# sahaRatul/sela

Hardware: AMD Instinct MI355X
Metric: Msamples/s encode+decode, 16-bit stereo 44.1kHz, 1/2/4/8 GPU; bit-exact vs CPU (higher is better)
Workload: dtype f64+int64

## Files before the change

### sela_amd/csrc/sela_encode.hip

```cpp
#include <algorithm>
#include <atomic>
#include <random>
#include <vector>

#include "sela_device.h"

namespace sela {

constexpr int kPadC = 64;
constexpr int kHalfEntries = kBlock / 4;
constexpr int kParityLen = kPadC + kHalfEntries + 64;
constexpr int kLastT0 = (kHalfEntries + 64) / 32 - 1;
constexpr int kFirstT1 = (kHalfEntries - kPadC) / 32;
constexpr int kRingHalf = 64;
constexpr int kRingLen = 2 * kRingHalf + 64;
constexpr int kRingsPerXcd = 512;
constexpr int kXcds = 8;
constexpr int kPadS = 128;
constexpr int kSBufWords = (kPadS + kBlock) / 32 * 33;
constexpr int kSmallBase = 8992;
constexpr int kBigBytes = kSmallBase + 3008;
static_assert(kResWordsCap * 4 <= kSmallBase, "packed residue words must fit the dead sample buffer");
static_assert(kSBufWords * 4 <= kSmallBase && kSmallBase % 16 == 0, "sample buffer must end below the analysis arrays");
static_assert(kBigBytes >= 2 * kParityLen * 8, "the FP64 parity arrays must fit");
// ... 909 lines not shown
#pragma unroll
    for (int t = 0; t <= kLastT0; t++)
        mine[half + 32 * t] = scale_sample(s[t]);
    wave_sync();

    __builtin_amdgcn_s_setprio(3);
    double sum = 0.0;
#pragma unroll 1
    for (int h = 0; h < 2; h++) {
        if (h == 1) {
            wave_sync();
#pragma unroll
            for (int t = kFirstT1; t < kPerLane; t++)
                mine1[half + 32 * t] = scale_sample(s[t]);
            wave_sync();
        }
        uint32_t addr = (uint32_t)(uintptr_t)(__attribute__((address_space(3))) double*)E;
        MeanFetch f0, f1;
        SELA_MEAN_ISSUE(f0, addr, 0, sum);
#pragma unroll 1
        for (int m0 = 0; m0 < kHalfEntries; m0 += 16) {
            mean_wait(f0, sum);
            SELA_MEAN_ISSUE(f1, addr, 64, sum);
            mean_steps(f0, sum);
            mean_wait(f1, sum);
            SELA_MEAN_ISSUE(f0, addr, 128, sum);
            mean_steps(f1, sum);
            addr += 128;
        }
        mean_wait(f0, sum);
    }
    mean = sum / (double)kBlock;
    __builtin_amdgcn_s_setprio(0);
    }

    SELA_STAMP(2);
    wave_sync();
    for (int m = lane; m < kPadC; m += 64) {
        E[m - kPadC] = 0.0;
        O[m - kPadC] = 0.0;
    }
#pragma unroll
    for (int t = 0; t <= kLastT0; t++)
        mine[half + 32 * t] = scale_sample(s[t]) - mean;
    wave_sync();

    SELA_STAMP(3);
    double acc_e = 0.0, acc_o = 0.0;
    {
        uint32_t xcc;
        asm volatile("s_getreg_b32 %0, hwreg(HW_REG_XCC_ID)" : "=s"(xcc));
        xcc &= kXcds - 1;
        uint32_t* const pool = ring_owner + xcc * kRingsPerXcd;
        uint32_t slot = 0;
        if (lane == 0) {
            slot = (e >> 3) & (kRingsPerXcd - 1);
            while (atomicExch(pool + slot, ticket) == ticket)
                slot = (slot + 1) & (kRingsPerXcd - 1);
        }
        slot = (uint32_t)__builtin_amdgcn_readfirstlane((int)slot);
        double* const ring = reinterpret_cast<double*>(
            read_first_lane((uint64_t)(rings + ((size_t)xcc * kRingsPerXcd + slot) * kRingLen)));
        __attribute__((address_space(1))) double* const ring_g = (__attribute__((address_space(1))) double*)ring;
        auto store_chunk = [&](int k, const double* resident) {
#pragma unroll
            for (int t = 0; t < kRingHalf / 64; t++) {
                const double c = resident[half + 32 * (t + (kRingHalf / 64) * k)];
                ring_g[(k & 1) * kRingHalf + lane + 64 * t] = c;
                if (t == 0 && !(k & 1) && lane < 16)
                    ring_g[2 * kRingHalf + lane] = c;
            }
        };
        store_chunk(0, mine);
        store_chunk(1, mine);
        asm volatile("s_waitcnt vmcnt(0)\n\ts_dcache_inv" ::: "memory");

        double A = E[-lane];
        double B = 0.0;
        uint32_t addr_e = (uint32_t)(uintptr_t)(__attribute__((address_space(3))) double*)(E - lane);
        uint32_t addr_o = (uint32_t)(uintptr_t)(__attribute__((address_space(3))) double*)(O - lane);
        const double* c_ptr = ring;
        AcFetch f0, f1;
        asm volatile("" : "+v"(A));
        SELA_AC_ISSUE_S(f0, c_ptr, 0, 64, acc_e, acc_o);
        SELA_AC_ISSUE_V(f0, addr_e, addr_o, 0, 1, 2, 3, 4, 5, 6, 7, 8, acc_e, acc_o);
        constexpr int kSwitch = kBlock / 2 / kRingHalf;
        const bool falling = !kFused && n_workers == 0 && fa.priorities != 0;
#pragma unroll 1
        for (int k = 0; k < kBlock / kRingHalf; k++) {
            if (falling && k == 0)
                __builtin_amdgcn_s_setprio(2);
            if (falling && k == kSwitch)
                __builtin_amdgcn_s_setprio(1);
            if (k == kSwitch) {
                wave_sync();
#pragma unroll
                for (int t = kFirstT1; t < kPerLane; t++)
                    mine1[half + 32 * t] = scale_sample(s[t]) - mean;
                wave_sync();
                addr_e -= kHalfEntries * 8;
                addr_o -= kHalfEntries * 8;
            }
            if (k >= 1 && k + 1 < kBlock / kRingHalf)
                store_chunk(k + 1, k >= kSwitch ? mine1 : mine);
#pragma unroll 1
            for (int it = 0; it < kRingHalf / 32; it++) {
                if (it == kRingHalf / 32 - 1)
                    asm volatile("s_waitcnt vmcnt(0)\n\ts_dcache_inv" ::: "memory");
                ac_wait(f0, acc_e, acc_o);
                SELA_AC_ISSUE_S(f1, c_ptr, 128, 192, acc_e, acc_o);
                ac_steps_head(f0, A, B, acc_e, acc_o);
                SELA_AC_ISSUE_V(f1, addr_e, addr_o, 8, 9, 10, 11, 12, 13, 14, 15, 16, acc_e, acc_o);
                ac_steps_tail(f0, A, B, acc_e, acc_o);
                ac_wait(f1, acc_e, acc_o);
                SELA_AC_ISSUE_S(f0, c_ptr, 256, 320, acc_e, acc_o);
                ac_steps_head(f1, A, B, acc_e, acc_o);
                SELA_AC_ISSUE_V(f0, addr_e, addr_o, 16, 17, 18, 19, 20, 21, 22, 23, 24, acc_e, acc_o);
                ac_steps_tail(f1, A, B, acc_e, acc_o);
                c_ptr += 32;
                addr_e += 128;
                addr_o += 128;
            }
            if (k & 1)
                c_ptr = ring;
        }
        ac_wait(f0, acc_e, acc_o);
        if (lane == 0)
            atomicExch(pool + slot, 0u);
    }
    wave_sync();

    SELA_STAMP(4);
    {
        const double ac0 = read_first_lane(acc_e);
        if (lane <= 50) {
            sm->ac[2 * lane] = lane == 0 ? 1.0 : acc_e / ac0;
            sm->ac[2 * lane + 1] = acc_o / ac0;
        }
    }
    wave_sync();

    double k_lo = 0.0, k_hi = 0.0;
    if (!kFused && n_workers == 0 && fa.priorities != 0)
        __builtin_amdgcn_s_setprio(1);
    else
        __builtin_amdgcn_s_setprio(2);
    {
        double g0a = sm->ac[lane + 1], g1a = g0a;
        double g0b = lane < 36 ? sm->ac[lane + 65] : 0.0, g1b = g0b;
        double err = 1.0;
        double g = read_first_lane(g1a);
        double ki = -g / err;
        err += g * ki;
        sm->k[0] = ki;
        constexpr int kTwoRegs = kMaxOrder - 64 + 1;
#pragma unroll 1
        for (int i = 1; i < kTwoRegs; i++) {
            const double sa = wave_shl1(read_first_lane(g1b), g1a);
            const double sb = wave_shl1_zero(g1b);
            g1a = sa + ki * g0a;
            g0a = sa * ki + g0a;
            g1b = sb + ki * g0b;
            g0b = sb * ki + g0b;
            g = read_first_lane(g1a);
            ki = -g / err;
            err += g * ki;
            sm->k[i] = ki;
        }
#pragma unroll 1
        for (int i = kTwoRegs; i < kMaxOrder; i++) {
            const double sa = wave_shl1_zero(g1a);
            g1a = sa + ki * g0a;
            g0a = sa * ki + g0a;
            g = read_first_lane(g1a);
            ki = -g / err;
            err += g * ki;
            sm->k[i] = ki;
        }
        wave_sync();
        k_lo = sm->k[lane];
        k_hi = lane < kMaxOrder - 64 ? sm->k[lane + 64] : 0.0;
        wave_sync();
    }
    if (kMode == 3) {
        uint64_t h_ac = hash_term(sm->ac[lane], lane) ^ (lane + 64 <= kMaxOrder ? hash_term(sm->ac[lane + 64], lane + 64) : 0ull);
        uint64_t h_k = hash_term(k_lo, lane) ^ (lane < kMaxOrder - 64 ? hash_term(k_hi, lane + 64) : 0ull);
        h_ac = lanes_xor<64>(h_ac);
        h_k = lanes_xor<64>(h_k);
        if (lane == 0) {
            uint64_t* const hp = reinterpret_cast<uint64_t*>(trace) + 2 * (size_t)block_id;
            hp[0] = h_ac;
            hp[1] = h_k;
        }
    }

    {
        constexpr bool kAcInLds = true;
        uint64_t* const sizes_pub = fa.sizes_pub;
        const uint64_t sizes_tag = fa.sizes_tag;
#define SELA_TAIL_TRACE_RESIDUES fa.trace_residues
#include "sela_encode_tail.inc"
#undef SELA_TAIL_TRACE_RESIDUES
    }
    SELA_STAMP(12);
    if (kFused) {
        const uint32_t g = frame / kGroupFrames;
        const uint32_t blocks_in_group = min((uint32_t)kGroupFrames, n_frames - g * kGroupFrames) * n_sig;
        stores_done();
        uint32_t last = 0;
        if (lane == 0)
            last = group_arrive(fa.group_count + (size_t)g * kGroupCountStride, fa.tag, blocks_in_group) ? 1u : 0u;
        if (__builtin_amdgcn_readfirstlane((int)last)) {
            drop_stale_lines();
            finish_group(fa, g, lane);
        }
    }
    SELA_STAMP(13);
    if (kMode == 2 && lane == 0)
        for (int i = 0; i < 13; i++)
            phase_cycles[(size_t)block_id * 16 + i] = (uint64_t)(stamp[i + 1] - stamp[i]);
}

constexpr int kTeamMirror = 24;
constexpr int kTeamWin = 16;
constexpr int kTeamAhead = 3;
constexpr int kTeamMeanChunk = 64;

template <int P>
struct TeamPlan {
    static constexpr int B = kWave / P;
    static constexpr int G = (kMaxOrder + 1 + P - 1) / P;
    static constexpr int kChunk = P == 8 ? 16 : 64;
    static constexpr int kRing = P == 8 ? 160 : 256;
    static constexpr int kStride = P == 8 ? kRing + kTeamMirror : kRing + 48;
    static constexpr int kPer = kChunk / P;
    static constexpr int kMeanPer = kTeamMeanChunk / P;
    static constexpr int kRingBytes = B * kStride * 8;
    static constexpr int kCwBase = kBigBytes;
    static constexpr int kKStride = 104;
    static constexpr int kQBase = kSmallBase;
    static constexpr int kQStride = 104;
    static constexpr int kLdsBytes = kRingBytes > kCwBase + kCoefWordsCap * 4 ? kRingBytes : kCwBase + kCoefWordsCap * 4;
    static_assert(G + kTeamAhead <= kTeamWin && kChunk % kTeamWin == 0 && kRing % kChunk == 0 && kStride % 32 == (P == 8 ? 24 : 16) && kStride >= kRing + kTeamMirror, "team plan");
    static_assert((G * P - 1) + kChunk + kChunk <= kRing && 2 * kTeamMeanChunk <= kRing, "the ring must hold the lags' reach, the chunk in use and the chunk being written");
    static_assert(kLdsBytes * 12 <= 160 * 1024, "twelve waves per CU");
    static_assert(B * kKStride * 8 <= kQBase && B * kKStride * 8 <= kRingBytes && B * kQStride <= 104 * 8, "k[] in the dead rings below the q store; the q store inside SmallArrays::ac");
};

template <int P>
__device__ __forceinline__ uint32_t team_first(uint32_t v)
{
    if constexpr (P == 16) {
        return (uint32_t)__builtin_amdgcn_mov_dpp((int)v, 0x150 , 0xf, 0xf, true);
    } else {
        static_assert(P == 8, "teams of 8 or 16 lanes");
        const int q = __builtin_amdgcn_mov_dpp((int)v, 0x00 , 0xf, 0xf, true);
        return (uint32_t)__builtin_amdgcn_update_dpp(q, q, 0x114 , 0xf, 0xa , false);
    }
}
template <int P>
__device__ __forceinline__ double team_first(double v)
{
    const uint64_t x = __builtin_bit_cast(uint64_t, v);
    return __builtin_bit_cast(double, ((uint64_t)team_first<P>((uint32_t)(x >> 32)) << 32) | team_first<P>((uint32_t)x));
}

template <int kPer, int kStep>
__device__ __forceinline__ void team_load_raw(const int16_t* __restrict__ fp, uint32_t channels, uint32_t sig, int first, int32_t (&raw)[kPer])
{
    if (channels == 2) {
        const uint32_t* pw = reinterpret_cast<const uint32_t*>(fp) + first;
        uint32_t w[kPer];
        if constexpr (kStep == 1 && kPer % 4 == 0) {
#pragma unroll
            for (int u = 0; u < kPer / 4; u++) {
                const uint4 v = reinterpret_cast<const uint4*>(pw)[u];
                w[4 * u] = v.x, w[4 * u + 1] = v.y, w[4 * u + 2] = v.z, w[4 * u + 3] = v.w;
            }
        } else if constexpr (kStep == 1 && kPer % 2 == 0) {
#pragma unroll
            for (int u = 0; u < kPer / 2; u++) {
                const uint2 v = reinterpret_cast<const uint2*>(pw)[u];
                w[2 * u] = v.x, w[2 * u + 1] = v.y;
            }
        } else {
#pragma unroll
            for (int u = 0; u < kPer; u++)
                w[u] = pw[u * kStep];
        }
        const uint32_t first_shift = sig == 1 ? 16u : 0u;
        const uint32_t second_mask = sig == 2 ? 0xFFFFFFFFu : 0u;
#pragma unroll
        for (int i = 0; i < kPer; i++) {
            const int32_t a = (int32_t)(w[i] << (16 - first_shift)) >> 16, b = ((int32_t)w[i] >> 16) & (int32_t)second_mask;
            raw[i] = a - b;
        }
    } else {
#pragma unroll
        for (int i = 0; i < kPer; i++)
            raw[i] = fp[(size_t)(first + i * kStep) * channels + sig];
    }
}

template <int kPer, int kStep, bool kCentre, bool kMirror, int kRing>
__device__ __forceinline__ void team_stage(double* ring_b, int pos, const int32_t (&raw)[kPer], double mean)
{
#pragma unroll
    for (int i = 0; i < kPer; i++) {
        const double x = scale_sample(raw[i]);
        const double c = kCentre ? x - mean : x;
        ring_b[pos + i * kStep] = c;
        if (kMirror && pos + i * kStep < kTeamMirror)
            ring_b[kRing + pos + i * kStep] = c;
    }
}

template <int kN>
__device__ __forceinline__ double team_chain(const double* x, double sum)
{
    constexpr int kBatch = 8;
    static_assert(kN % (2 * kBatch) == 0, "two batches per round");
    double u[kBatch], v[kBatch];
#pragma unroll
    for (int i = 0; i < kBatch; i++)
        u[i] = x[i];
#pragma unroll
    for (int i0 = 0; i0 < kN; i0 += 2 * kBatch) {
#pragma unroll
        for (int i = 0; i < kBatch; i++)
            v[i] = x[i0 + kBatch + i];
        __builtin_amdgcn_sched_barrier(0);
#pragma unroll
        for (int i = 0; i < kBatch; i++)
            sum += u[i];
        __builtin_amdgcn_sched_barrier(0);
        if (i0 + 2 * kBatch < kN) {
#pragma unroll
            for (int i = 0; i < kBatch; i++)
                u[i] = x[i0 + 2 * kBatch + i];
        }
        __builtin_amdgcn_sched_barrier(0);
#pragma unroll
        for (int i = 0; i < kBatch; i++)
            sum += v[i];
        __builtin_amdgcn_sched_barrier(0);
    }
    return sum;
}

template <int G, int R0>
__device__ __forceinline__ void team_ac_steps(double (&W)[kTeamWin], double (&M)[4], double (&acc)[G], uint32_t addr_w, uint32_t addr_m)
{
    asm volatile("ds_read_b64 %0, %2 offset:%4\n\tds_read_b64 %1, %3 offset:%4"
                 : "=&v"(W[(R0 + kTeamAhead) & (kTeamWin - 1)]), "=&v"(M[(R0 + kTeamAhead) & 3])
                 : "v"(addr_w), "v"(addr_m), "n"(8 * (R0 + kTeamAhead)), "v"(acc[0]), "v"(acc[G - 1])
                 : "memory");
    asm volatile("s_waitcnt lgkmcnt(6)" : "+v"(W[R0 & (kTeamWin - 1)]), "+v"(M[R0 & 3]));
    const double m = M[R0 & 3];
    constexpr int kAheadOps = 5;
#pragma unroll
    for (int g0 = 0; g0 < G; g0 += kAheadOps) {
        double t[kAheadOps];
#pragma unroll
        for (int u = 0; u < kAheadOps; u++)
            if (g0 + u < G)
                t[u] = m * W[(R0 - g0 - u) & (kTeamWin - 1)];
#pragma unroll
        for (int u = 0; u < kAheadOps; u++)
            if (g0 + u < G)
                acc[g0 + u] += t[u];
    }
    __builtin_amdgcn_sched_barrier(0);
    if constexpr (R0 < kTeamWin - 1)
        team_ac_steps<G, R0 + 1>(W, M, acc, addr_w, addr_m);
}

template <int kMode, int P>
__global__ __launch_bounds__(64) __attribute__((amdgpu_waves_per_eu(3, 3))) void k_encode_teams(
    const int16_t* __restrict__ pcm, uint32_t n_frames, uint32_t channels, uint32_t n_sig, BlockMeta* __restrict__ meta,
    uint32_t* __restrict__ slots, sela_hip_trace* __restrict__ trace, int force_plain_fir, uint64_t* __restrict__ phase_cycles,
    uint64_t* __restrict__ sizes_pub, uint64_t sizes_tag, uint32_t team_priorities)
{
    using Plan = TeamPlan<P>;
    constexpr int B = Plan::B, G = Plan::G, kPer = Plan::kPer, kMeanPer = Plan::kMeanPer, kChunk = Plan::kChunk, kRing = Plan::kRing;
    constexpr bool kTrace = kMode == 1;
    constexpr bool kFused = false;
    constexpr int kStep = P == 16 ? P : 1;
    __shared__ __attribute__((aligned(32))) unsigned char lds[Plan::kLdsBytes];
    unsigned char* const big = lds;
    uint32_t* const cw_buf = reinterpret_cast<uint32_t*>(lds + Plan::kCwBase);

    const int lane0 = threadIdx.x;
    const int b = lane0 / P, p = lane0 % P;
    const uint32_t wq = blockIdx.x % 8, wv = blockIdx.x / 8;
    const uint32_t sig = wv % n_sig;
    const uint32_t frame0 = ((wv / n_sig) * 8 + wq) * B;
    constexpr uint32_t frame_stride = 1;
    if (frame0 >= n_frames)
        return;
    const bool team_live = frame0 + (uint32_t)b * frame_stride < n_frames;
    const uint32_t my_frame = team_live ? frame0 + (uint32_t)b * frame_stride : frame0;
    const int16_t* const fp = pcm + (size_t)my_frame * kBlock * channels;
    double* const ring_b = reinterpret_cast<double*>(lds) + b * Plan::kStride;
    double* const k_b = reinterpret_cast<double*>(lds) + b * Plan::kKStride;
    long long wave_stamp[5];
    if (kMode == 2)
        wave_stamp[0] = clock64();

    double mean;
    {
        constexpr int kChunks = kBlock / kTeamMeanChunk;
        const int mine = kStep == 1 ? p * kMeanPer : p;
        int32_t raw_a[kMeanPer], raw_b[kMeanPer];
        team_load_raw<kMeanPer, kStep>(fp, channels, sig, mine, raw_a);
        team_stage<kMeanPer, kStep, false, false, kRing>(ring_b, mine, raw_a, 0.0);
        team_load_raw<kMeanPer, kStep>(fp, channels, sig, kTeamMeanChunk + mine, raw_a);
        team_load_raw<kMeanPer, kStep>(fp, channels, sig, 2 * kTeamMeanChunk + mine, raw_b);
        double sum = 0.0;
        const uint32_t quarter_priorities = team_priorities;
        set_wave_priority((int)(quarter_priorities & 0xFF));
#pragma unroll 1
        for (int c = 0; c < kChunks; c++) {
            const int here = (c & 1) * kTeamMeanChunk, there = kTeamMeanChunk - here;
            if (c + 1 < kChunks)
                team_stage<kMeanPer, kStep, false, false, kRing>(ring_b, there + mine, raw_a, 0.0);
#pragma unroll
            for (int i = 0; i < kMeanPer; i++)
                raw_a[i] = raw_b[i];
            if (c + 3 < kChunks)
                team_load_raw<kMeanPer, kStep>(fp, channels, sig, (c + 3) * kTeamMeanChunk + mine, raw_b);
            wave_sync();
            sum = team_chain<kTeamMeanChunk>(ring_b + here, sum);
            wave_sync();
        }
        mean = sum / (double)kBlock;
    }
    if (kMode == 2)
        wave_stamp[1] = clock64();

    double acc[G];
    {
#pragma unroll
        for (int g = 0; g < G; g++)
            acc[g] = 0.0;
        for (int i = kChunk + p; i < Plan::kStride; i += P)
            ring_b[i] = 0.0;
        const int mine = kStep == 1 ? p * kPer : p;
        int32_t raw_a[kPer], raw_b[kPer];
        team_load_raw<kPer, kStep>(fp, channels, sig, mine, raw_a);
        team_stage<kPer, kStep, true, true, kRing>(ring_b, mine, raw_a, mean);
        team_load_raw<kPer, kStep>(fp, channels, sig, kChunk + mine, raw_a);
        team_load_raw<kPer, kStep>(fp, channels, sig, 2 * kChunk + mine, raw_b);
        wave_sync();
        const uint32_t ring_addr = (uint32_t)(uintptr_t)(__attribute__((address_space(3))) double*)ring_b;
        double W[kTeamWin], M[4];
#pragma unroll
        for (int i = 0; i < kTeamWin; i++)
            W[i] = 0.0;
        uint32_t idx_w = (uint32_t)((kRing - G * p) % kRing);
        uint32_t idx_m = 0, pos_stage = kChunk;
        uint32_t addr_w = ring_addr + 8 * idx_w, addr_m = ring_addr;
        asm volatile("ds_read_b64 %0, %6\n\tds_read_b64 %3, %7\n\t"
                     "ds_read_b64 %1, %6 offset:8\n\tds_read_b64 %4, %7 offset:8\n\t"
                     "ds_read_b64 %2, %6 offset:16\n\tds_read_b64 %5, %7 offset:16"
                     : "=&v"(W[0]), "=&v"(W[1]), "=&v"(W[2]), "=&v"(M[0]), "=&v"(M[1]), "=&v"(M[2])
                     : "v"(addr_w), "v"(addr_m)
                     : "memory");
        M[3] = 0.0;
        constexpr int kChunks = kBlock / kChunk;
        auto trips = [&]() {
#pragma unroll 1
            for (int it = 0; it < kChunk / kTeamWin; it++) {
                team_ac_steps<G, 0>(W, M, acc, addr_w, addr_m);
                idx_w += kTeamWin;
                idx_w = idx_w >= (uint32_t)kRing ? idx_w - kRing : idx_w;
                idx_m += kTeamWin;
                idx_m = idx_m >= (uint32_t)kRing ? idx_m - kRing : idx_m;
                addr_w = ring_addr + 8 * idx_w;
                addr_m = ring_addr + 8 * idx_m;
            }
        };
        auto stage_next = [&](const int32_t (&raw)[kPer]) {
            team_stage<kPer, kStep, true, true, kRing>(ring_b, (int)pos_stage + mine, raw, mean);
            pos_stage += kChunk;
            pos_stage = pos_stage >= (uint32_t)kRing ? 0u : pos_stage;
        };
        constexpr int kPrio2From = (int)(0.27 * kChunks), kPrio1From = (int)(0.71 * kChunks);
#pragma unroll 1
        for (int c = 0; c < kChunks; c++) {
            if (c == kPrio2From)
                set_wave_priority((int)((team_priorities >> 8) & 0xFF));
            if (c == kPrio1From)
                set_wave_priority((int)((team_priorities >> 16) & 0xFF));
            if (c + 1 < kChunks)
                stage_next(raw_a);
#pragma unroll
            for (int i = 0; i < kPer; i++)
                raw_a[i] = raw_b[i];
            if (c + 3 < kChunks)
                team_load_raw<kPer, kStep>(fp, channels, sig, (c + 3) * kChunk + mine, raw_b);
            trips();
        }
        asm volatile("s_waitcnt lgkmcnt(0)" : "+v"(W[0]), "+v"(W[1]), "+v"(W[2]), "+v"(M[0]), "+v"(M[1]), "+v"(M[2]));
    }
    wave_sync();
    if (kMode == 2)
        wave_stamp[2] = clock64();

    {
        const double ac0 = team_first<P>(acc[0]);
#pragma unroll
        for (int g = 0; g < G; g++)
            acc[g] = (p == 0 && g == 0) ? 1.0 : acc[g] / ac0;
    }
    if (kTrace && team_live) {
        sela_hip_trace* tr = trace + (size_t)my_frame * n_sig + sig;
        if (p == 0)
            tr->mean = mean;
#pragma unroll
        for (int g = 0; g < G; g++)
            if (G * p + g <= kMaxOrder)
                tr->ac[G * p + g] = acc[g];
    }
    if (kMode == 3) {
        uint64_t h = 0;
#pragma unroll
        for (int g = 0; g < G; g++)
            h ^= G * p + g <= kMaxOrder ? hash_term(acc[g], G * p + g) : 0ull;
        h = lanes_xor<P>(h);
        if (team_live && p == 0)
            reinterpret_cast<uint64_t*>(trace)[2 * ((size_t)my_frame * n_sig + sig)] = h;
    }

    {
        double g0[G], g1[G];
        const double next_first = wave_shl1_zero(acc[0]);
#pragma unroll
        for (int r = 0; r < G; r++) {
            const double v = r + 1 < G ? acc[r + 1] : next_first;
            g0[r] = g1[r] = (G * p + r < kMaxOrder) ? v : 0.0;
        }
        double err = 1.0;
        const bool keeper = p == 0;
        double g = team_first<P>(g1[0]);
        double ki = -g / err;
        err += g * ki;
        if (keeper)
            k_b[0] = ki;
#pragma unroll 1
        for (int i = 1; i < kMaxOrder; i++) {
            const double crossing = wave_shl1_zero(g1[0]);
#pragma unroll
            for (int r = 0; r < G; r++) {
                const double sa = r + 1 < G ? g1[r + 1] : crossing;
                g1[r] = sa + ki * g0[r];
                g0[r] = sa * ki + g0[r];
            }
            g = team_first<P>(g1[0]);
            ki = -g / err;
            err += g * ki;
            if (keeper)
                k_b[i] = ki;
        }
    }
    wave_sync();
    if (kMode == 2)
        wave_stamp[3] = clock64();

    int8_t* const q_all = reinterpret_cast<int8_t*>(lds + Plan::kQBase);
#pragma unroll 1
    for (int bb = 0; bb < B; bb++) {
        const uint32_t frame = frame0 + (uint32_t)bb * frame_stride;
        if (frame >= n_frames)
            break;
        int lane_now = lane0;
        asm volatile("" : "+v"(lane_now));
        const int lane = lane_now;
        const double* const k_mine = reinterpret_cast<const double*>(lds) + bb * Plan::kKStride;
        const double k_lo = k_mine[lane];
        const double k_hi = lane < kMaxOrder - 64 ? k_mine[64 + lane] : 0.0;
        int order;
        {
            const unsigned long long b_lo = __ballot(fabs(k_lo) > SELA_ORDER_THRESHOLD);
            const unsigned long long b_hi = __ballot(lane < 36 && fabs(k_hi) > SELA_ORDER_THRESHOLD);
            order = b_hi ? 128 - __clzll(b_hi) : (b_lo ? 64 - __clzll(b_lo) : 1);
        }
        const double sqrt2 = SELA_SQRT2;
        double v_lo;
        if (lane == 0)
            v_lo = floor(64 * (-1 + (sqrt2 * sqrt(k_lo + 1))));
        else if (lane == 1)
            v_lo = floor(64 * (-1 + (sqrt2 * sqrt(-k_lo + 1))));
        else
            v_lo = floor(64 * k_lo);
        const double v_hi = floor(64 * k_hi);
        const int32_t q_lo = isnan(v_lo) ? 0 : (int32_t)v_lo;
        const int32_t q_hi = isnan(v_hi) ? 0 : (int32_t)v_hi;
        const bool wide = (lane < order && (q_lo < -128 || q_lo > 127)) || (lane + 64 < order && (q_hi < -128 || q_hi > 127));
        const bool escape = __any(wide);
        int8_t* const q_mine = q_all + bb * Plan::kQStride;
        q_mine[lane] = (int8_t)q_lo;
        if (lane < kMaxOrder - 64)
            q_mine[64 + lane] = (int8_t)q_hi;
        if (lane == 0) {
            q_mine[100] = (int8_t)order;
            q_mine[101] = escape ? 1 : 0;
        }
        if (escape) {
            int32_t* const q_wide = reinterpret_cast<int32_t*>(slots + ((size_t)frame * n_sig + sig) * kSlotWords);
            q_wide[lane] = q_lo;
            if (lane < kMaxOrder - 64)
                q_wide[64 + lane] = q_hi;
        }
        if (kTrace) {
            sela_hip_trace* tr = trace + (size_t)frame * n_sig + sig;
            tr->k[lane] = k_lo;
            if (lane < 36)
                tr->k[lane + 64] = k_hi;
        }
        if (kMode == 3) {
            uint64_t h = hash_term(k_lo, lane) ^ (lane < kMaxOrder - 64 ? hash_term(k_hi, lane + 64) : 0ull);
            h = lanes_xor<64>(h);
            if (lane == 0)
                reinterpret_cast<uint64_t*>(trace)[2 * ((size_t)frame * n_sig + sig) + 1] = h;
        }
    }
    wave_sync();

    SmallArrays* const sm = reinterpret_cast<SmallArrays*>(big + kSmallBase);
    long long stamp[14];
#pragma unroll 1
    for (int bb = 0; bb < B; bb++) {
        const uint32_t frame = frame0 + (uint32_t)bb * frame_stride;
        if (frame >= n_frames)
            break;
        int lane_now = lane0;
        asm volatile("" : "+v"(lane_now));
        const int lane = lane_now;
        const uint32_t block_id = frame * n_sig + sig;
        if (4 * (bb + 1) > B)
            set_wave_priority((int)((team_priorities >> 24) & 0xFF));
        const int8_t* const q_mine = q_all + bb * Plan::kQStride;
        const int order = (uint8_t)q_mine[100];
        int32_t q_lo = q_mine[lane], q_hi = lane < kMaxOrder - 64 ? q_mine[64 + lane] : 0;
        if (__builtin_amdgcn_readfirstlane((int)q_mine[101])) {
            const int32_t* const q_wide = reinterpret_cast<const int32_t*>(slots + (size_t)block_id * kSlotWords);
            q_lo = q_wide[lane];
            q_hi = lane < kMaxOrder - 64 ? q_wide[64 + lane] : 0;
        }
        const double mean = 0.0;
        int32_t s[kPerLane];
        {
            const int16_t* fb = pcm + (size_t)frame * kBlock * channels;
            if (channels == 2) {
                const uint32_t* fp2 = reinterpret_cast<const uint32_t*>(fb);
#pragma unroll
                for (int t = 0; t < kPerLane; t++) {
                    const uint32_t w = fp2[lane + 64 * t];
                    const int32_t l = (int16_t)(w & 0xFFFFu), r = (int16_t)(w >> 16);
                    s[t] = sig == 0 ? l : (sig == 1 ? r : l - r);
                }
            } else {
#pragma unroll
                for (int t = 0; t < kPerLane; t++)
                    s[t] = fb[(size_t)(lane + 64 * t) * channels + sig];
            }
        }
        uint32_t flags = 0;
        wave_sync();
        {
            constexpr bool kAcInLds = false;
#define SELA_TAIL_HAVE_Q
#include "sela_encode_tail.inc"
#undef SELA_TAIL_HAVE_Q
        }
        SELA_STAMP(12);
        if (kMode == 2 && lane == 0) {
            uint64_t* row = phase_cycles + (size_t)block_id * 16;
            const long long now = clock64();
            row[0] = 0;
            row[1] = (uint64_t)(wave_stamp[1] - wave_stamp[0]);
            row[2] = 0;
            row[3] = (uint64_t)(wave_stamp[2] - wave_stamp[1]);
            row[4] = (uint64_t)(wave_stamp[3] - wave_stamp[2]);
            for (int i = 5; i < 12; i++)
                row[i] = (uint64_t)(stamp[i + 1] - stamp[i]);
            row[12] = (uint64_t)(now - wave_stamp[3]);
            row[13] = (uint64_t)wave_stamp[0];
            row[14] = (uint64_t)now;
        }
    }
}

constexpr int kPlanThreadsBig = 1024, kPlanFramesBig = 12288;
constexpr int kPlanThreadsSmall = 256, kPlanFramesSmall = 4096;

template <int kPlanThreads, int kPlanLdsFrames>
__global__ __launch_bounds__(kPlanThreads) void k_plan_frames(const BlockMeta* __restrict__ meta, uint32_t n_frames,
    uint32_t channels, uint32_t n_sig, size_t frames_cap, uint64_t* frame_offsets,
    uint8_t* __restrict__ choice_out, uint32_t* __restrict__ status,
    const uint64_t* base_in ,
    uint32_t accumulate )
{
    __shared__ uint64_t part[kPlanThreads / kWave];
    __shared__ uint32_t frame_size[kPlanLdsFrames];
    __shared__ uint32_t acc[2];
    __shared__ uint64_t start;
    const uint32_t tid = threadIdx.x;
    if (tid < 2)
        acc[tid] = 0;
    if (tid == 0)
        start = base_in ? *base_in : 0;
    __syncthreads();
// ... 449 lines not shown
```

Baseline: 16370.

## Compute team mean with DPP row broadcast FMAC chains for 16-lane teams

For 16-lane teams, the mean is now computed directly in registers. Each lane fetches its strided samples and accumulates the whole row's sum via v_fmac_f64_dpp with row_newbcast over all 16 lanes, in the sequential order the bit-exact result requires. This bypasses the LDS staging and the serial LDS read chain used before. The trade is 16 DPP FMACs per element per lane instead of LDS traffic, and the summation order must still match the CPU reference exactly.

Measured after the change: 16660 (median of 6 runs). +1.8%, better.

```diff
diff --git a/sela_amd/csrc/sela_encode.hip b/sela_amd/csrc/sela_encode.hip
--- a/sela_amd/csrc/sela_encode.hip
+++ b/sela_amd/csrc/sela_encode.hip
@@ -1235,6 +1235,38 @@
     }
 }
 
+template <int kPer, int kStep, bool kStereo>
+__device__ __forceinline__ void team_fetch(const int16_t* __restrict__ fp, uint32_t channels, uint32_t sig, int first, uint32_t (&w)[kPer])
+{
+    if constexpr (kStereo) {
+        const uint32_t* pw = reinterpret_cast<const uint32_t*>(fp) + first;
+#pragma unroll
+        for (int u = 0; u < kPer; u++)
+            w[u] = pw[u * kStep];
+    } else {
+#pragma unroll
+        for (int i = 0; i < kPer; i++)
+            w[i] = (uint32_t)(int32_t)fp[(size_t)(first + i * kStep) * channels + sig];
+    }
+}
+template <int kPer, bool kStereo>
+__device__ __forceinline__ void team_unpack(uint32_t sig, const uint32_t (&w)[kPer], int32_t (&raw)[kPer])
+{
+    if constexpr (kStereo) {
+        const uint32_t first_shift = sig == 1 ? 16u : 0u;
+        const uint32_t second_mask = sig == 2 ? 0xFFFFFFFFu : 0u;
+#pragma unroll
+        for (int i = 0; i < kPer; i++) {
+            const int32_t a = (int32_t)(w[i] << (16 - first_shift)) >> 16, b = ((int32_t)w[i] >> 16) & (int32_t)second_mask;
+            raw[i] = a - b;
+        }
+    } else {
+#pragma unroll
+        for (int i = 0; i < kPer; i++)
+            raw[i] = (int32_t)w[i];
+    }
+}
+
 template <int kPer, int kStep, bool kCentre, bool kMirror, int kRing>
 __device__ __forceinline__ void team_stage(double* ring_b, int pos, const int32_t (&raw)[kPer], double mean)
 {
@@ -1276,6 +1308,58 @@
 #pragma unroll
         for (int i = 0; i < kBatch; i++)
             sum += v[i];
+        __builtin_amdgcn_sched_barrier(0);
+    }
+    return sum;
+}
+
+template <int kN>
+__device__ __forceinline__ double row_chain(const double (&x)[kN], double sum)
+{
+#define SELA_ROW_FMAC(j) "v_fmac_f64_dpp %0, %1, %2 row_newbcast:" #j "\n\t"
+#pragma unroll
+    for (int i = 0; i < kN; i++)
+        asm("s_nop 1\n\t" SELA_ROW_FMAC(0) SELA_ROW_FMAC(1) SELA_ROW_FMAC(2) SELA_ROW_FMAC(3) SELA_ROW_FMAC(4) SELA_ROW_FMAC(5)
+            SELA_ROW_FMAC(6) SELA_ROW_FMAC(7) SELA_ROW_FMAC(8) SELA_ROW_FMAC(9) SELA_ROW_FMAC(10) SELA_ROW_FMAC(11) SELA_ROW_FMAC(12)
+            SELA_ROW_FMAC(13) SELA_ROW_FMAC(14) SELA_ROW_FMAC(15)
+            : "+v"(sum) : "v"(x[i]), "v"(1.0));
+#undef SELA_ROW_FMAC
+    return sum;
+}
+
+template <int kPer, bool kStereo>
+__device__ __forceinline__ double team_row_mean_sum(const int16_t* __restrict__ fp, uint32_t channels, uint32_t sig, int p)
+{
+    constexpr int kStep = 16, kChunks = kBlock / kTeamMeanChunk;
+    static_assert(kPer * kStep == kTeamMeanChunk && kChunks % 2 == 0, "lane p holds samples p, p + 16, .. of a chunk; two chunks per trip");
+    uint32_t w_a[kPer], w_b[kPer];
+    double x[kPer];
+    int32_t raw[kPer];
+    team_fetch<kPer, kStep, kStereo>(fp, channels, sig, p, w_a);
+    team_unpack<kPer, kStereo>(sig, w_a, raw);
+#pragma unroll
+    for (int i = 0; i < kPer; i++)
+        x[i] = scale_sample(raw[i]);
+    team_fetch<kPer, kStep, kStereo>(fp, channels, sig, kTeamMeanChunk + p, w_a);
+    team_fetch<kPer, kStep, kStereo>(fp, channels, sig, 2 * kTeamMeanChunk + p, w_b);
+    double sum = 0.0;
+#pragma unroll 1
+    for (int c = 0; c < kChunks; c += 2) {
+        sum = row_chain<kPer>(x, sum);
+        __builtin_amdgcn_sched_barrier(0);
+        team_unpack<kPer, kStereo>(sig, w_a, raw);
+#pragma unroll
+        for (int i = 0; i < kPer; i++)
+            x[i] = scale_sample(raw[i]);
+        team_fetch<kPer, kStep, kStereo>(fp, channels, sig, min(c + 3, kChunks - 1) * kTeamMeanChunk + p, w_a);
+        __builtin_amdgcn_sched_barrier(0);
+        sum = row_chain<kPer>(x, sum);
+        __builtin_amdgcn_sched_barrier(0);
+        team_unpack<kPer, kStereo>(sig, w_b, raw);
+#pragma unroll
+        for (int i = 0; i < kPer; i++)
+            x[i] = scale_sample(raw[i]);
+        team_fetch<kPer, kStep, kStereo>(fp, channels, sig, min(c + 4, kChunks - 1) * kTeamMeanChunk + p, w_b);
         __builtin_amdgcn_sched_barrier(0);
     }
     return sum;
@@ -1341,7 +1425,12 @@
         wave_stamp[0] = clock64();
 
     double mean;
-    {
+    if constexpr (P == 16) {
+        static_assert(kStep == P, "lane p holds samples p, p + 16, .. of a chunk");
+        set_wave_priority((int)(team_priorities & 0xFF));
+        const double sum = channels == 2 ? team_row_mean_sum<kMeanPer, true>(fp, channels, sig, p) : team_row_mean_sum<kMeanPer, false>(fp, channels, sig, p);
+        mean = sum / (double)kBlock;
+    } else {
         constexpr int kChunks = kBlock / kTeamMeanChunk;
         const int mine = kStep == 1 ? p * kMeanPer : p;
         int32_t raw_a[kMeanPer], raw_b[kMeanPer];
```
